# marbl/parsnp

Measured on AMD Instinct MI355X. Metric: genomes/sec (MUM+LCB end-to-end), higher is better.
Workload: dtype int32

## Files before the change

### parsnp_amd/csrc/engine/kernels.h

```cpp
#pragma once
#include <cstdint>

#if defined(__HIPCC__)
#define PM_HD __host__ __device__ inline
#else
#define PM_HD inline
#endif

namespace pm {

PM_HD int ctz64(uint64_t x) {
#if defined(__HIP_DEVICE_COMPILE__)
    return __ffsll((unsigned long long)x) - 1;
#else
    return __builtin_ctzll(x);
#endif
}
PM_HD int clz64(uint64_t x) {
#if defined(__HIP_DEVICE_COMPILE__)
    return __clzll((long long)x);
#else
    return __builtin_clzll(x);
#endif
}
// ... 844 lines not shown
        uint64_t* ev_count = ev_counters + slice * kSliceStride;
        const uint64_t ev_cap = slice_cap;
        uint64_t* const key_out = ev_key + slice * slice_cap;
        uint64_t* const val_out = ev_val + slice * slice_cap;
        uint64_t bk = kEmpty, bv = 0;
        auto emit = [&](int strand, int32_t l0, int64_t j0, int32_t len) {
            const uint64_t ek = ((((uint64_t)pair << lbits) | (uint64_t)l0) << 1) | (uint64_t)strand;
            const uint64_t evv = ((uint64_t)j0 << 32) | (uint32_t)len;
            if (bk == kEmpty) { bk = ek; bv = evv; }
            else { const uint64_t at = atomic_add64(ev_count, 1); if (at < ev_cap) { key_out[at] = ek; val_out[at] = evv; } }
        };
        auto reverse_seed = [&](int64_t j, int32_t l) {
            const int64_t jr = m - K - j;
            const int64_t qpr = rec.qbase_r + jr;
            int32_t lim = (int32_t)(jr < l ? jr : l);
            if (lim > stride) lim = stride;
            const int32_t left = lce_bwd(P, qpr, rbase + l, lim);
            if (left >= stride) return;
            const int32_t rep_l0 = rep[ri.posbase + l - left];
            const int32_t rr = ri.nR - l - K;
            const int32_t maxr = (int32_t)(j < rr ? j : rr);
            const int32_t right = lce_fwd(P, qpr + K, rbase + l + K, maxr);
            const int32_t len = left + K + right;
            if (len >= ri.minlen && len > rep_l0) emit(1, l - left, jr - left, len);
        };
        auto forward_seed = [&](int64_t j, int32_t l) {
            int32_t lim = (int32_t)(j < l ? j : l);
            if (lim > stride) lim = stride;
            const int32_t left = lce_bwd(P, qbase + j, rbase + l, lim);
            if (left >= stride) return;
            const int32_t rep_l0 = rep[ri.posbase + l - left];
            const int64_t mr = m - j - K; const int32_t rr = ri.nR - l - K;
            const int32_t maxr = (int32_t)(mr < rr ? mr : rr);
            const int32_t right = lce_fwd64(P, qbase + j + K, rbase + l + K, maxr);
            const int32_t len = left + K + right;
            if (len >= ri.minlen && len > rep_l0) emit(0, l - left, j - left, len);
        };
        auto walk = [&](int64_t j, uint64_t tag, uint64_t gat, uint64_t slot, int32_t skip, uint64_t head_rt) {
            const bool multi = (slot & kMulti) != 0;
            const int32_t head = slot_head(slot);
            for (int32_t l = head; l >= 0; l = multi ? next[ri.posbase + l] : -1) {
                if (++work > budget) { atomic_or32(err, kErrWork); dense[rec.region] = 1; return; }
                if (l == skip) continue;
                const uint64_t rt = l == head ? head_rt : kmer_tag(P, rbase + l, K);
                if (rt == tag) forward_seed(j, l);
                if (rt == gat) reverse_seed(j, l);
            }
        };
        auto probe_sample = [&](int64_t j, uint64_t tag, uint64_t gat) {
            const uint64_t ctag = gat < tag ? gat : tag;
            uint64_t slot = index_probe(ri, slots, filter, ctag);
            if (slot == kEmpty) return;
            uint64_t rt = kmer_tag(P, rbase + slot_head(slot), K);
            if (rt != tag && rt != gat) {
                slot = index_lookup(P, ri, slots, filter, ctag);
                if (slot == kEmpty) return;
                rt = kmer_tag(P, rbase + slot_head(slot), K);
            }
            walk(j, tag, gat, slot, -1, rt);
        };

        if (live) {
            const int64_t j = (int64_t)it.sample * stride;
            if (it.l >= 0) reverse_seed(j, it.l);
            else if (!dense[rec.region]) {
                const uint64_t tg = kmer_tag(P, qbase + j, K);
                probe_sample(j, tg, rc_tag(tg, K));
            }
        }
        const uint64_t at = wave_reserve01(ev_count, bk != kEmpty);
        if (bk != kEmpty && at < ev_cap) { key_out[at] = bk; val_out[at] = bv; }
    }
};

PM_HD uint64_t even_bits(uint64_t x) {
    x &= 0x5555555555555555ull;
    x = (x | (x >> 1)) & 0x3333333333333333ull;
    x = (x | (x >> 2)) & 0x0f0f0f0f0f0f0f0full;
    x = (x | (x >> 4)) & 0x00ff00ff00ff00ffull;
    x = (x | (x >> 8)) & 0x0000ffff0000ffffull;
    x = (x | (x >> 16)) & 0x00000000ffffffffull;
    return x;
}
PM_HD void planes64(const SeqBlock* blk, int64_t p, uint64_t* b0, uint64_t* b1, uint64_t* nm) {
    const SeqBlock* b = blk + (p >> 5);
    const int sh = (int)(p & 31);
    const SeqBlock x0 = b[0], x1 = b[1], x2 = b[2];
    const uint64_t lo = (x0.b2 >> (2 * sh)) | ((x1.b2 << 1) << (63 - 2 * sh));
    const uint64_t hi = (x1.b2 >> (2 * sh)) | ((x2.b2 << 1) << (63 - 2 * sh));
    *b0 = even_bits(lo) | (even_bits(hi) << 32);
    *b1 = even_bits(lo >> 1) | (even_bits(hi >> 1) << 32);
    const uint64_t m01 = (uint64_t)x0.nm | ((uint64_t)x1.nm << 32);
    *nm = (m01 >> sh) | (((uint64_t)x2.nm << 1) << (63 - sh));
}
struct W64 {
    uint64_t v;
    static PM_HD W64 load(const SeqBlock* blk, int64_t p, int plane) {
        uint64_t b0, b1, nm; planes64(blk, p, &b0, &b1, &nm);
        W64 w; w.v = plane == 0 ? b0 : plane == 1 ? b1 : nm; return w;
    }
    static PM_HD W64 ones(int n) { W64 w; w.v = n >= 64 ? ~0ull : ((1ull << n) - 1); return w; }
    PM_HD W64 shr(int k) const { W64 w; w.v = v >> k; return w; }
    PM_HD W64 operator^(const W64& o) const { W64 w; w.v = v ^ o.v; return w; }
    PM_HD W64 operator|(const W64& o) const { W64 w; w.v = v | o.v; return w; }
    PM_HD W64 operator&(const W64& o) const { W64 w; w.v = v & o.v; return w; }
    PM_HD W64 operator~() const { W64 w; w.v = ~v; return w; }
    PM_HD bool any() const { return v != 0; }
    PM_HD int low() const { return ctz64(v); }
    PM_HD int run_at(int s) const { const uint64_t t = ~(v >> s); return t ? ctz64(t) : 64 - s; }
    PM_HD W64 clear_below(int k) const { W64 w; w.v = k >= 64 ? 0 : v & (~0ull << k); return w; }
    static constexpr int kBits = 64;
};
struct W128 {
    uint64_t lo, hi;
    static PM_HD W128 load(const SeqBlock* blk, int64_t p, int plane) {
        uint64_t a0, a1, an, c0, c1, cn; planes64(blk, p, &a0, &a1, &an); planes64(blk, p + 64, &c0, &c1, &cn);
        W128 w; w.lo = plane == 0 ? a0 : plane == 1 ? a1 : an; w.hi = plane == 0 ? c0 : plane == 1 ? c1 : cn; return w;
    }
    static PM_HD W128 ones(int n) {
        W128 w;
        w.lo = n >= 64 ? ~0ull : ((1ull << n) - 1);
        w.hi = n >= 128 ? ~0ull : n > 64 ? ((1ull << (n - 64)) - 1) : 0;
        return w;
    }
    PM_HD W128 shr(int k) const {
        W128 w;
        if (k >= 64) { w.lo = k >= 128 ? 0 : hi >> (k - 64); w.hi = 0; }
        else { w.lo = (lo >> k) | ((hi << 1) << (63 - k)); w.hi = hi >> k; }
        return w;
    }
    PM_HD W128 operator^(const W128& o) const { W128 w; w.lo = lo ^ o.lo; w.hi = hi ^ o.hi; return w; }
    PM_HD W128 operator|(const W128& o) const { W128 w; w.lo = lo | o.lo; w.hi = hi | o.hi; return w; }
    PM_HD W128 operator&(const W128& o) const { W128 w; w.lo = lo & o.lo; w.hi = hi & o.hi; return w; }
    PM_HD W128 operator~() const { W128 w; w.lo = ~lo; w.hi = ~hi; return w; }
    PM_HD bool any() const { return (lo | hi) != 0; }
    PM_HD int low() const { return lo ? ctz64(lo) : 64 + ctz64(hi); }
    PM_HD int run_at(int s) const { const W128 t = ~shr(s); return t.any() ? t.low() : 128 - s; }
    PM_HD W128 clear_below(int k) const {
        W128 w;
        if (k >= 128) { w.lo = 0; w.hi = 0; }
        else if (k >= 64) { w.lo = 0; w.hi = hi & (~0ull << (k - 64)); }
        else { w.lo = lo & (~0ull << k); w.hi = hi; }
        return w;
    }
    static constexpr int kBits = 128;
};

template <class W, class Emit>
PM_HD void pair_diagonals(const Packed& P, int64_t rpos, int64_t qpos, int32_t nR, int32_t m, int32_t L, Emit emit, int32_t first = 0, int32_t step = 1) {
    const W r0 = W::load(P.blk, rpos, 0), r1 = W::load(P.blk, rpos, 1), rn = W::load(P.blk, rpos, 2);
    const W q0 = W::load(P.blk, qpos, 0), q1 = W::load(P.blk, qpos, 1), qn = W::load(P.blk, qpos, 2);
    const W vr = W::ones(nR), vq = W::ones(m);
    for (int32_t d = -(m - L) + first; d <= nR - L; d += step) {
        W eq;
        if (d >= 0) eq = ~((r0.shr(d) ^ q0) | (r1.shr(d) ^ q1) | (rn.shr(d) ^ qn)) & vr.shr(d) & vq;
        else eq = ~((r0 ^ q0.shr(-d)) | (r1 ^ q1.shr(-d)) | (rn ^ qn.shr(-d))) & vr & vq.shr(-d);
        W x = eq;
        int k = 1;
        while (2 * k <= L) { x = x & x.shr(k); k *= 2; }
        if (L > k) x = x & x.shr(L - k);
        if (!x.any()) continue;
        while (eq.any()) {
            const int s = eq.low();
            const int len = eq.run_at(s);
            if (len >= L) emit(d >= 0 ? s + d : s, d >= 0 ? s : s - d, len);
            eq = eq.clear_below(s + len);
        }
    }
}
struct SmallPairEvents {
    Packed P; const RegionInfo* R; const int64_t* starts; const int64_t* lens; int32_t ngen;
    const int32_t* rep;
    uint64_t* ev_key; uint64_t* ev_val; uint64_t* ev_counters; uint64_t slice_cap; int lbits;
    int32_t g_first, g_last;
    const uint8_t* grouped;

    template <class W, class Emit>
    PM_HD void scan(int64_t rpos, int64_t qpos, int32_t nR, int32_t m, int32_t L, Emit emit) const { pair_diagonals<W>(P, rpos, qpos, nR, m, L, emit); }

    PM_HD void operator()(int64_t tid) const {
        const int64_t pair = tid >> 1; const int strand = (int)(tid & 1);
        const int32_t nq = ngen - 1;
        const int64_t r = pair / nq; const int g = (int)(pair % nq) + 1;
        const RegionInfo& ri = R[r];
        const bool mine = !(grouped && grouped[r]);
        const int64_t m = mine ? lens[r * ngen + g] : 0, qs = mine ? starts[r * ngen + g] : 0;
        const int32_t nR = ri.nR, L = ri.minlen;
        const uint64_t slice = (uint64_t)((tid >> 8) & (kSlices - 1));
        uint64_t* ev_count = ev_counters + slice * kSliceStride;
        uint64_t* const key_out = ev_key + slice * slice_cap;
        uint64_t* const val_out = ev_val + slice * slice_cap;
        uint64_t first_key = kEmpty, first_val = 0;
        if (mine && small_pair(nR, m) && m >= L && nR >= L && g >= g_first && g < g_last) {
            const int64_t qbase = strand ? P.goff[2 * g + 1] + (P.glen[g] - qs - m) : P.goff[2 * g] + qs;
            const int64_t rbase = P.goff[0] + ri.ref_pos;
            auto emit = [&](int32_t l0, int32_t j0, int32_t len) {
                if (len <= rep[ri.posbase + l0]) return;
                const uint64_t ek = ((((uint64_t)pair << lbits) | (uint64_t)l0) << 1) | (uint64_t)strand;
                const uint64_t evv = ((uint64_t)j0 << 32) | (uint32_t)len;
                if (first_key == kEmpty) { first_key = ek; first_val = evv; }
                else { const uint64_t at = atomic_add64(ev_count, 1); if (at < slice_cap) { key_out[at] = ek; val_out[at] = evv; } }
            };
            if (nR <= 64 && m <= 64) scan<W64>(rbase, qbase, nR, (int32_t)m, L, emit);
            else scan<W128>(rbase, qbase, nR, (int32_t)m, L, emit);
        }
        const uint64_t at = wave_reserve01(ev_count, first_key != kEmpty);
        if (first_key != kEmpty && at < slice_cap) { key_out[at] = first_key; val_out[at] = first_val; }
    }
};

struct SliceOffsets {
    const uint64_t* counters; int64_t* off;
    PM_HD void wave(int64_t) const {
#if defined(__HIP_DEVICE_COMPILE__)
        const int lane = (int)__lane_id();
        constexpr int per = kSlices / 64;
        int64_t c[per]; int64_t sum = 0;
        for (int i = 0; i < per; i++) { c[i] = (int64_t)counters[(size_t)(lane * per + i) * kSliceStride]; sum += c[i]; }
        int64_t run = wave_incl_sum64(sum) - sum;
        for (int i = 0; i < per; i++) { off[lane * per + i] = run; run += c[i]; }
        if (lane == 63) off[kSlices] = run;
#else
        int64_t run = 0;
        for (int i = 0; i < kSlices; i++) { off[i] = run; run += (int64_t)counters[(size_t)i * kSliceStride]; }
        off[kSlices] = run;
#endif
    }
};
struct CompactEvents {
    const uint64_t* key_in; const uint64_t* val_in; const int64_t* off; uint64_t slice_cap; uint64_t* key_out; uint64_t* val_out;
    PM_HD void operator()(int64_t tid) const {
        int64_t sl = upper_slot(off, kSlices, tid);
        int64_t src = sl * (int64_t)slice_cap + (tid - off[sl]);
        key_out[tid] = key_in[src]; val_out[tid] = val_in[src];
    }
};

struct PairBucketBase {
    int32_t nq; const int64_t* cbase; int64_t* pbase;
    PM_HD void operator()(int64_t pair) const {
        const int64_t r = pair / nq; const int64_t g = pair % nq;
        pbase[pair] = (int64_t)nq * (cbase[r] - r) + g * (cbase[r + 1] - cbase[r] - 1);
    }
};
PM_HD int64_t bucket_of_key(uint64_t k, int lbits, const int64_t* pbase) {
    return pbase[k >> (lbits + 1)] + (int64_t)(((k >> 1) & ((1ull << lbits) - 1)) >> 8);
}
struct EventBucketCount {
    const uint64_t* key_in; const uint64_t* counters; uint64_t slice_cap; int shift; int lbits; const int64_t* pbase; int64_t* count;
    PM_HD void operator()(int64_t tid) const {
        const uint64_t sl = (uint64_t)tid >> shift, idx = (uint64_t)tid & ((1ull << shift) - 1);
// ... 695 lines not shown
```

### parsnp_amd/csrc/engine/store_kernels.h

```cpp
#pragma once
#include "kernels.h"

namespace pm {

#if defined(__HIP_DEVICE_COMPILE__)
template <class F> __device__ inline void lanes_for(int from, int n, F f) {
    for (int j = (from & ~63) + (int)__lane_id(); j < n; j += 64) if (j >= from) f(j);
}
__device__ inline int32_t wave_min_i32(int32_t x) { for (int d = 32; d >= 1; d >>= 1) { const int32_t y = __shfl_xor(x, d, 64); if (y < x) x = y; } return x; }
__device__ inline int32_t wave_max_i32(int32_t x) { for (int d = 32; d >= 1; d >>= 1) { const int32_t y = __shfl_xor(x, d, 64); if (y > x) x = y; } return x; }
__device__ inline uint32_t wave_or_u32(uint32_t x) { for (int d = 32; d >= 1; d >>= 1) x |= (uint32_t)__shfl_xor((int)x, d, 64); return x; }
__device__ inline int32_t wave_bcast_i32(int32_t x, int lane) { return __shfl(x, lane, 64); }
__device__ inline uint64_t wave_or_u64(uint64_t x) { return ((uint64_t)wave_or_u32((uint32_t)(x >> 32)) << 32) | wave_or_u32((uint32_t)x); }
__device__ inline uint64_t wave_sum_u64(uint64_t x) {
    for (int d = 32; d >= 1; d >>= 1) x += ((uint64_t)(uint32_t)__shfl_xor((int)(x >> 32), d, 64) << 32) | (uint32_t)__shfl_xor((int)(uint32_t)x, d, 64);
    return x;
}
__device__ inline bool wave_leader() { return __lane_id() == 0; }
__device__ inline void wave_sync() { __syncthreads(); }
#define PM_WAVE_SHARED __shared__
__device__ inline uint64_t load_coherent64(const uint64_t* p) { return __hip_atomic_load(p, __ATOMIC_RELAXED, __HIP_MEMORY_SCOPE_AGENT); }
__device__ inline int32_t load_coherent32(const int32_t* p) { return __hip_atomic_load(p, __ATOMIC_RELAXED, __HIP_MEMORY_SCOPE_AGENT); }
__device__ inline uint8_t load_coherent8(const uint8_t* p) { return __hip_atomic_load(p, __ATOMIC_RELAXED, __HIP_MEMORY_SCOPE_AGENT); }
__device__ inline void store_coherent32(int32_t* p, int32_t v) { __hip_atomic_store(p, v, __ATOMIC_RELAXED, __HIP_MEMORY_SCOPE_AGENT); }
// ... 540 lines not shown
        const int64_t i = xcd_item(w, rows);
        if (i >= rows || i >= *nacc || !keep[i]) return;
        const int64_t c = acc[i];
        const int32_t dl = S.shift[c], len = S.len[c];
        const int n = S.ngen;
        int64_t slot = off[i];
        for (int side = 0; side < 2; side++) {
            if (!(keep[i] & (1 << side))) continue;
            if ((uint64_t)slot >= cap) return;
            int64_t rs, rl;
            const int32_t smin = region_extent(S, L, P, c, dl, len, side, &rs, &rl);
            lanes_for(0, n, [&](int j) {
                int64_t a, b;
                region_side(S, L, P, c, dl, len, side, j, &a, &b);
                rg_start[slot * n + j] = a; rg_len[slot * n + j] = b - a;
            });
            if (wave_leader()) info[slot] = RegInfo{2 * i + side, rs, rl, smin, (int32_t)c};
            slot++;
        }
    }
};
constexpr int kAlgPairs = 256;
constexpr int kAlgSets = 64;
struct AlgBytes {
    const RegionInfo* R; const int64_t* lens; int32_t ngen; int64_t npairs; uint64_t* out;
    PM_HD void wave(int64_t w) const {
        uint64_t a = 0, k = 0, q = 0;
        lanes_for(0, kAlgPairs, [&](int t) {
            const int64_t pair = w * kAlgPairs + t;
            if (pair >= npairs) return;
            const int64_t r = pair / (ngen - 1); const int g = (int)(pair % (ngen - 1)) + 1;
            const RegionInfo& ri = R[r];
            const int64_t m = lens[r * ngen + g], n = ri.nR;
            a += (uint64_t)(65 * m + 64 * n);
            k += (uint64_t)m + (g == 1 ? (uint64_t)n : 0ull);
            if (!(m <= 128 && n <= 128) && m >= ri.K && n >= ri.K) k += 16ull * (uint64_t)((m - ri.K) / ri.stride + 1);
            q += (uint64_t)m;
        });
        a = wave_sum_u64(a); k = wave_sum_u64(k); q = wave_sum_u64(q);
        uint64_t* set = out + (size_t)(w & (kAlgSets - 1)) * 8;
        if (wave_leader()) { atomic_add64(set, a); atomic_add64(set + 1, k); atomic_add64(set + 2, q); }
    }
};
struct GatherRegions {
    const int32_t* ids; int32_t ngen; const int64_t* rg_start; const int64_t* rg_len; int64_t* starts; int64_t* lens;
    PM_HD void operator()(int64_t tid) const {
        const int64_t r = ids[tid / ngen]; const int j = (int)(tid % ngen);
        starts[tid] = rg_start[r * ngen + j]; lens[tid] = rg_len[r * ngen + j];
    }
};
struct RegionsEqual {
    const int32_t* a; const int32_t* b; int32_t ngen; const int64_t* rg_start; const int64_t* rg_len; uint8_t* same;
    PM_HD void wave(int64_t i) const {
        const int64_t x = a[i], y = b[i];
        uint32_t diff = 0;
        lanes_for(0, ngen, [&](int j) { if (rg_start[x * ngen + j] != rg_start[y * ngen + j] || rg_len[x * ngen + j] != rg_len[y * ngen + j]) diff = 1; });
        diff = wave_or_u32(diff);
        if (wave_leader()) same[i] = diff ? 0 : 1;
    }
};

#ifndef PM_GRP_EVENTS
#define PM_GRP_EVENTS 8
#endif
constexpr int kGrpEvents = PM_GRP_EVENTS;
constexpr int kGrpPieces = 32;
constexpr int kGrpGenomes = 1024;
struct GroupedPairEvents {
    Packed P; const RegionInfo* R; const int64_t* starts; const int64_t* lens; int32_t ngen; const int32_t* rep;
    uint64_t* ev_key; uint64_t* ev_val; uint64_t* block_count; uint64_t ev_cap; int lbits; int64_t* glo; int32_t g_first, g_last;
    uint8_t* flag;
    EventAtK* st; int32_t* emax;
    int32_t* epm;
    int64_t nreg;
    PM_HD void wave(int64_t w) const {
        const int64_t r = xcd_item(w, nreg);
        if (r >= nreg) return;
        const int32_t nq = ngen - 1;
        const int per = (nq + 63) / 64;
        const RegionInfo& ri = R[r];
        const int32_t nR = ri.nR, L = ri.minlen;
        const int64_t rbase = P.goff[0] + ri.ref_pos;
        uint32_t big = nR > 128 ? 1u : 0u;
        lanes_for(1, ngen, [&](int g) { if (lens[r * ngen + g] > 128) big = 1; });
        big = wave_or_u32(big);
        if (big) { if (wave_leader()) flag[r] = 0; return; }
        PM_WAVE_SHARED uint64_t sh_pl[64][6];
        PM_WAVE_SHARED int32_t sh_m[64];
        PM_WAVE_SHARED uint8_t sh_open[64];
        PM_WAVE_SHARED uint64_t rp_pl[kGrpPieces][6];
        PM_WAVE_SHARED int32_t rp_m[kGrpPieces];
        PM_WAVE_SHARED int32_t rp_g[kGrpPieces];
        PM_WAVE_SHARED uint8_t sh_piece[kGrpGenomes];
        PM_WAVE_SHARED uint32_t sh_ev[2 * kGrpPieces][kGrpEvents];
        PM_WAVE_SHARED int32_t sh_cnt[2 * kGrpPieces];
        PM_WAVE_SHARED uint32_t sh_st[2 * kGrpPieces][kGrpEvents];
        PM_WAVE_SHARED uint8_t sh_used[kGrpPieces];
        PM_WAVE_SHARED int32_t sh_tot[64];
        PM_WAVE_SHARED int32_t sh_elect;
        PM_WAVE_SHARED int32_t sh_bad;
        PM_WAVE_SHARED uint64_t sh_base;
        if (wave_leader()) sh_bad = 0;
        lanes_for(0, kGrpPieces, [&](int i) { sh_used[i] = 0; });
        int npieces = 0;
        for (int k = 0; k < per; k++) {
            wave_sync();
            lanes_for(0, 64, [&](int t) {
                const int g = 1 + t * per + k;
                int32_t m = -1;
                if (g < ngen) {
                    m = (int32_t)lens[r * ngen + g];
                    const int64_t qpos = P.goff[2 * g] + starts[r * ngen + g];
                    const W128 v = W128::ones(m);
                    for (int pl = 0; pl < 3; pl++) { const W128 x = W128::load(P.blk, qpos, pl) & v; sh_pl[t][2 * pl] = x.lo; sh_pl[t][2 * pl + 1] = x.hi; }
                }
                sh_m[t] = m;
                uint8_t open = m >= 0;
                for (int i = 0; i < npieces && open; i++) {
                    if (rp_m[i] != m) continue;
                    bool same = true;
                    for (int x = 0; x < 6 && same; x++) same = rp_pl[i][x] == sh_pl[t][x];
                    if (same) { sh_piece[g - 1] = (uint8_t)i; open = 0; }
                }
                sh_open[t] = open;
            });
            for (;;) {
                wave_sync();
                if (wave_leader()) sh_elect = 64;
                wave_sync();
                lanes_for(0, 64, [&](int t) { if (sh_open[t]) lds_min32(&sh_elect, t); });
                wave_sync();
                const int e = sh_elect;
                if (e == 64) break;
                if (npieces == kGrpPieces) { if (wave_leader()) sh_bad = 1; break; }
                lanes_for(0, 64, [&](int t) {
                    if (t != e) return;
                    for (int x = 0; x < 6; x++) rp_pl[npieces][x] = sh_pl[t][x];
                    rp_m[npieces] = sh_m[t]; rp_g[npieces] = 1 + t * per + k;
                });
                wave_sync();
                lanes_for(0, 64, [&](int t) {
                    if (!sh_open[t] || rp_m[npieces] != sh_m[t]) return;
                    bool same = true;
                    for (int x = 0; x < 6 && same; x++) same = rp_pl[npieces][x] == sh_pl[t][x];
                    if (same) { sh_piece[t * per + k] = (uint8_t)npieces; sh_open[t] = 0; }
                });
                npieces++;
            }
            wave_sync();
            if (sh_bad) break;
        }
        const int tasks = 2 * npieces;
        int share = 1;
        while (share * 2 * tasks <= 64) share *= 2;
        if (!sh_bad) {
            lanes_for(0, tasks, [&](int wi) { sh_cnt[wi] = 0; });
            wave_sync();
            lanes_for(0, tasks * share, [&](int t) {
                const int wi = t / share, sub = t % share;
                const int g = rp_g[wi >> 1], strand = wi & 1;
                const int32_t m = rp_m[wi >> 1];
                if (m < L || nR < L) return;
                const int64_t qs = starts[r * ngen + g];
                const int64_t qbase = strand ? P.goff[2 * g + 1] + (P.glen[g] - qs - m) : P.goff[2 * g] + qs;
                auto emit = [&](int32_t l0, int32_t j0, int32_t len) {
                    if (len <= rep[ri.posbase + l0]) return;
                    const int32_t at = lds_add32(&sh_cnt[wi], 1);
                    if (at < kGrpEvents) sh_ev[wi][at] = (uint32_t)l0 | ((uint32_t)j0 << 8) | ((uint32_t)len << 16);
                };
                if (nR <= 64 && m <= 64) pair_diagonals<W64>(P, rbase, qbase, nR, m, L, emit, sub, share);
                else pair_diagonals<W128>(P, rbase, qbase, nR, m, L, emit, sub, share);
            });
            wave_sync();
            lanes_for(0, tasks, [&](int wi) {
                const int n = sh_cnt[wi];
                if (n > kGrpEvents) { sh_bad = 1; return; }
                for (int i = 1; i < n; i++) {
                    const uint32_t e = sh_ev[wi][i];
                    int at = i;
                    while (at > 0 && (sh_ev[wi][at - 1] & 0xffu) > (e & 0xffu)) { sh_ev[wi][at] = sh_ev[wi][at - 1]; at--; }
                    sh_ev[wi][at] = e;
                }
            });
        }
        wave_sync();
        if (sh_bad) { if (wave_leader()) flag[r] = 0; return; }
        lanes_for(0, tasks, [&](int wi) {
            const int n = sh_cnt[wi];
            int32_t e1 = 0, e2 = 0, wl = 0, wj = 0, up = 0; bool have = false;
            for (int i = 0; i < n; i++) {
                const uint32_t e = sh_ev[wi][i];
                const int32_t l = (int32_t)(e & 0xffu), j = (int32_t)((e >> 8) & 0xffu), end = l + (int32_t)(e >> 16);
                const bool take = !have || end > e1 || (end == e1 && (l < wl || (l == wl && j < wj)));
                if (take) { if (have && e1 > e2) e2 = e1; e1 = end; wl = l; wj = j; up = l + rep[ri.posbase + l]; have = true; }
                else if (end > e2) e2 = end;
                sh_st[wi][i] = (uint32_t)e1 | ((uint32_t)(e2 > up ? e2 : up) << 8) | ((uint32_t)(wj - wl + 128) << 16);
            }
        });
        lanes_for(0, 64, [&](int t) {
            int c = 0;
            for (int k = 0; k < per; k++) {
                const int g = 1 + t * per + k;
                if (g < ngen && g >= g_first && g < g_last) { const int i = sh_piece[g - 1]; c += sh_cnt[2 * i] + sh_cnt[2 * i + 1]; sh_used[i] = 1; }
            }
            sh_tot[t] = c;
        });
        wave_sync();
        lanes_for(0, nR, [&](int k) {
            int32_t ep = nR;
            for (int i = 0; i < npieces; i++) {
                if (!sh_used[i]) continue;
                int32_t v = 0;
                for (int sd = 0; sd < 2; sd++) {
                    const int wi = 2 * i + sd, n = sh_cnt[wi];
                    int32_t e = 0;
                    for (int x = 0; x < n && (int32_t)(sh_ev[wi][x] & 0xffu) <= k; x++) e = (int32_t)(sh_st[wi][x] & 0xffu);
                    if (e > v) v = e;
                }
                if (v < ep) ep = v;
            }
            epm[ri.posbase + k] = ep;
        });
        if (wave_leader()) {
            int total = 0;
            for (int t = 0; t < 64; t++) { const int c = sh_tot[t]; sh_tot[t] = total; total += c; }
            sh_base = total ? atomic_add64(block_count, (uint64_t)total) : 0;
            flag[r] = 1;
        }
        wave_sync();
        lanes_for(0, 64, [&](int t) {
            uint64_t at0 = sh_base + (uint64_t)sh_tot[t];
            for (int k = 0; k < per; k++) {
                const int g = 1 + t * per + k;
                if (g >= ngen) break;
                const int64_t pair = r * nq + (g - 1);
                glo[pair] = (int64_t)at0;
                if (g < g_first || g >= g_last) continue;
                const int i = sh_piece[g - 1];
                const uint32_t* a = sh_ev[2 * i]; const uint32_t* b = sh_ev[2 * i + 1];
                const int na = sh_cnt[2 * i], nb = sh_cnt[2 * i + 1], c = na + nb;
                if (at0 + (uint64_t)c <= ev_cap) {
                    int ia = 0, ib = 0;
                    for (int x = 0; x < c; x++) {
                        const bool fwd = ib >= nb || (ia < na && (a[ia] & 0xffu) <= (b[ib] & 0xffu));
                        const uint32_t e = fwd ? a[ia++] : b[ib++];
                        ev_key[at0 + x] = ((((uint64_t)pair << lbits) | (uint64_t)(e & 0xffu)) << 1) | (fwd ? 0ull : 1ull);
                        ev_val[at0 + x] = ((uint64_t)((e >> 8) & 0xffu) << 32) | (uint64_t)(e >> 16);
                        const uint32_t sf = ia ? sh_st[2 * i][ia - 1] : 0, sr = ib ? sh_st[2 * i + 1][ib - 1] : 0;
                        EventAtK o;
                        o.s[0] = sf ? StrandAtK{(int32_t)(sf & 0xffu), (int32_t)((sf >> 8) & 0xffu), (int32_t)(sf >> 16) - 128} : StrandAtK{0, 0, 0};
                        o.s[1] = sr ? StrandAtK{(int32_t)(sr & 0xffu), (int32_t)((sr >> 8) & 0xffu), (int32_t)(sr >> 16) - 128} : StrandAtK{0, 0, 0};
                        st[at0 + x] = o;
                        emax[at0 + x] = o.s[0].e1 > o.s[1].e1 ? o.s[0].e1 : o.s[1].e1;
                    }
                }
                at0 += (uint64_t)c;
            }
        });
    }
};
struct GroupedBounds {
    const uint8_t* flag; const int64_t* glo; int32_t nq; int64_t* lo;
    PM_HD void operator()(int64_t pair) const { if (flag[pair / nq]) lo[pair] = glo[pair]; }
};

constexpr int kWideEvents = 32;
constexpr int kWidePieces = 128;
constexpr int kWideGenomes = 2047;
struct GroupedPairEventsWide {
    Packed P; const RegionInfo* R; const int64_t* starts; const int64_t* lens; int32_t ngen; const int32_t* rep;
    uint64_t* ev_key; uint64_t* ev_val; uint64_t* block_count; uint64_t ev_cap; int lbits; int64_t* glo; int32_t g_first, g_last;
    uint8_t* flag;
    EventAtK* st; int32_t* emax; int32_t* epm;
    int64_t nreg;
    int after_first;
    uint64_t* wide;
    PM_HD void wave(int64_t w) const {
        const int64_t r = xcd_item(w, nreg);
        if (r >= nreg) return;
        if (after_first && flag[r]) return;
        const int32_t nq = ngen - 1;
        const int per = (nq + 63) / 64;
        const RegionInfo& ri = R[r];
        const int32_t nR = ri.nR, L = ri.minlen;
        const int64_t rbase = P.goff[0] + ri.ref_pos;
        uint32_t big = nR > 128 || nq > kWideGenomes ? 1u : 0u;
        lanes_for(1, ngen, [&](int g) { if (lens[r * ngen + g] > 128) big = 1; });
        big = wave_or_u32(big);
        if (big) { if (wave_leader()) flag[r] = 0; return; }
        PM_WAVE_SHARED uint64_t sh_pl[64][6];
        PM_WAVE_SHARED int32_t sh_m[64];
        PM_WAVE_SHARED uint8_t sh_open[64];
        PM_WAVE_SHARED uint64_t rp_pl[kWidePieces][6];
        PM_WAVE_SHARED int32_t rp_m[kWidePieces];
        PM_WAVE_SHARED int32_t rp_g[kWidePieces];
        PM_WAVE_SHARED uint8_t sh_piece[kWideGenomes + 1];
        PM_WAVE_SHARED uint32_t sh_ev[2 * kWidePieces][kWideEvents];
        PM_WAVE_SHARED int32_t sh_cnt[2 * kWidePieces];
        PM_WAVE_SHARED uint8_t sh_used[kWidePieces];
        PM_WAVE_SHARED int32_t sh_tot[64];
        PM_WAVE_SHARED int32_t sh_elect;
        PM_WAVE_SHARED int32_t sh_bad;
        PM_WAVE_SHARED uint64_t sh_base;
        if (wave_leader()) sh_bad = 0;
        lanes_for(0, kWidePieces, [&](int i) { sh_used[i] = 0; });
        int npieces = 0;
        bool bad = false;
        for (int k = 0; k < per && !bad; k++) {
            wave_sync();
            lanes_for(0, 64, [&](int t) {
                const int g = 1 + t * per + k;
                int32_t m = -1;
                if (g < ngen) {
                    m = (int32_t)lens[r * ngen + g];
                    const int64_t qpos = P.goff[2 * g] + starts[r * ngen + g];
                    const W128 v = W128::ones(m);
                    for (int pl = 0; pl < 3; pl++) { const W128 x = W128::load(P.blk, qpos, pl) & v; sh_pl[t][2 * pl] = x.lo; sh_pl[t][2 * pl + 1] = x.hi; }
                }
                sh_m[t] = m;
                uint8_t open = m >= 0;
                for (int i = 0; i < kWidePieces; i++) {
                    if (i >= npieces || !open) break;
                    if (rp_m[i] != m) continue;
                    bool same = true;
                    for (int x = 0; x < 6; x++) same = same && rp_pl[i][x] == sh_pl[t][x];
                    if (same) { sh_piece[g - 1] = (uint8_t)i; open = 0; }
                }
                sh_open[t] = open;
            });
            for (int round = 0; round < 65; round++) {
                wave_sync();
                if (wave_leader()) sh_elect = 64;
                wave_sync();
                lanes_for(0, 64, [&](int t) { if (sh_open[t]) lds_min32(&sh_elect, t); });
                wave_sync();
                const int e = sh_elect;
                if (e == 64) break;
                if (npieces == kWidePieces) { if (wave_leader()) sh_bad = 1; break; }
                lanes_for(0, 64, [&](int t) {
                    if (t != e) return;
// ... 1077 lines not shown
```

Before: 31370.

## Restructure grouped pair-events kernel: register planes, prefetch, LDS reuse, parallel output write

The grouped small-region event kernel now keeps each lane's query bit-planes in registers instead of LDS, and software-prefetches the next genome's sequence blocks. Diagonal scanning reuses the cached distinct-piece planes, deriving the reverse strand by bit reversal instead of reloading from global memory. The reference planes are loaded once, and repeat thresholds are staged into an LDS byte table. The event output loop now precomputes the merge order per piece and writes one event per lane using a wave prefix sum and binary search, replacing the serial per-lane merge. This adds complexity and relies on repeat values clamped to 255 and on correct bit-reversal equivalence for reverse strands.

```diff
diff --git a/parsnp_amd/csrc/engine/kernels.h b/parsnp_amd/csrc/engine/kernels.h
--- a/parsnp_amd/csrc/engine/kernels.h
+++ b/parsnp_amd/csrc/engine/kernels.h
@@ -950,16 +950,17 @@
     x = (x | (x >> 16)) & 0x00000000ffffffffull;
     return x;
 }
-PM_HD void planes64(const SeqBlock* blk, int64_t p, uint64_t* b0, uint64_t* b1, uint64_t* nm) {
-    const SeqBlock* b = blk + (p >> 5);
-    const int sh = (int)(p & 31);
-    const SeqBlock x0 = b[0], x1 = b[1], x2 = b[2];
+PM_HD void planes64_of(const SeqBlock& x0, const SeqBlock& x1, const SeqBlock& x2, int sh, uint64_t* b0, uint64_t* b1, uint64_t* nm) {
     const uint64_t lo = (x0.b2 >> (2 * sh)) | ((x1.b2 << 1) << (63 - 2 * sh));
     const uint64_t hi = (x1.b2 >> (2 * sh)) | ((x2.b2 << 1) << (63 - 2 * sh));
     *b0 = even_bits(lo) | (even_bits(hi) << 32);
     *b1 = even_bits(lo >> 1) | (even_bits(hi >> 1) << 32);
     const uint64_t m01 = (uint64_t)x0.nm | ((uint64_t)x1.nm << 32);
     *nm = (m01 >> sh) | (((uint64_t)x2.nm << 1) << (63 - sh));
+}
+PM_HD void planes64(const SeqBlock* blk, int64_t p, uint64_t* b0, uint64_t* b1, uint64_t* nm) {
+    const SeqBlock* b = blk + (p >> 5);
+    planes64_of(b[0], b[1], b[2], (int)(p & 31), b0, b1, nm);
 }
 struct W64 {
     uint64_t v;
@@ -1015,10 +1016,8 @@
 };
 
 template <class W, class Emit>
-PM_HD void pair_diagonals(const Packed& P, int64_t rpos, int64_t qpos, int32_t nR, int32_t m, int32_t L, Emit emit, int32_t first = 0, int32_t step = 1) {
-    const W r0 = W::load(P.blk, rpos, 0), r1 = W::load(P.blk, rpos, 1), rn = W::load(P.blk, rpos, 2);
-    const W q0 = W::load(P.blk, qpos, 0), q1 = W::load(P.blk, qpos, 1), qn = W::load(P.blk, qpos, 2);
-    const W vr = W::ones(nR), vq = W::ones(m);
+PM_HD void pair_diagonals(const W& r0, const W& r1, const W& rn, const W& q0, const W& q1, const W& qn, const W& vr, const W& vq,
+                          int32_t nR, int32_t m, int32_t L, Emit emit, int32_t first = 0, int32_t step = 1) {
     for (int32_t d = -(m - L) + first; d <= nR - L; d += step) {
         W eq;
         if (d >= 0) eq = ~((r0.shr(d) ^ q0) | (r1.shr(d) ^ q1) | (rn.shr(d) ^ qn)) & vr.shr(d) & vq;
@@ -1035,6 +1034,32 @@
             eq = eq.clear_below(s + len);
         }
     }
+}
+template <class W, class Emit>
+PM_HD void pair_diagonals(const Packed& P, int64_t rpos, int64_t qpos, int32_t nR, int32_t m, int32_t L, Emit emit, int32_t first = 0, int32_t step = 1) {
+    const W r0 = W::load(P.blk, rpos, 0), r1 = W::load(P.blk, rpos, 1), rn = W::load(P.blk, rpos, 2);
+    const W q0 = W::load(P.blk, qpos, 0), q1 = W::load(P.blk, qpos, 1), qn = W::load(P.blk, qpos, 2);
+    pair_diagonals<W>(r0, r1, rn, q0, q1, qn, W::ones(nR), W::ones(m), nR, m, L, emit, first, step);
+}
+PM_HD uint64_t rev_bits64(uint64_t x) {
+#if defined(__HIP_DEVICE_COMPILE__)
+    return (uint64_t)__brevll((unsigned long long)x);
+#else
+    x = ((x >> 1) & 0x5555555555555555ull) | ((x & 0x5555555555555555ull) << 1);
+    x = ((x >> 2) & 0x3333333333333333ull) | ((x & 0x3333333333333333ull) << 2);
+    x = ((x >> 4) & 0x0f0f0f0f0f0f0f0full) | ((x & 0x0f0f0f0f0f0f0f0full) << 4);
+    return __builtin_bswap64(x);
+#endif
+}
+PM_HD W128 reversed_bits(const W128& x, int32_t m) {
+    W128 w; w.lo = rev_bits64(x.hi); w.hi = rev_bits64(x.lo);
+    return w.shr(128 - m);
+}
+PM_HD void reverse_strand_planes(W128* b0, W128* b1, W128* nm, int32_t m) {
+    const W128 n = reversed_bits(*nm, m), keep = ~n & W128::ones(m);
+    *b0 = ~reversed_bits(*b0, m) & keep;
+    *b1 = ~reversed_bits(*b1, m) & keep;
+    *nm = n;
 }
 struct SmallPairEvents {
     Packed P; const RegionInfo* R; const int64_t* starts; const int64_t* lens; int32_t ngen;
diff --git a/parsnp_amd/csrc/engine/store_kernels.h b/parsnp_amd/csrc/engine/store_kernels.h
--- a/parsnp_amd/csrc/engine/store_kernels.h
+++ b/parsnp_amd/csrc/engine/store_kernels.h
@@ -646,68 +646,111 @@
         const int32_t nR = ri.nR, L = ri.minlen;
         const int64_t rbase = P.goff[0] + ri.ref_pos;
         uint32_t big = nR > 128 ? 1u : 0u;
-        lanes_for(1, ngen, [&](int g) { if (lens[r * ngen + g] > 128) big = 1; });
+        lanes_for(1, ngen, [&](int g) { const int64_t m = lens[r * ngen + g]; if (m > 128) big |= 1; if (m > 64) big |= 2; });
         big = wave_or_u32(big);
-        if (big) { if (wave_leader()) flag[r] = 0; return; }
-        PM_WAVE_SHARED uint64_t sh_pl[64][6];
-        PM_WAVE_SHARED int32_t sh_m[64];
-        PM_WAVE_SHARED uint8_t sh_open[64];
-        PM_WAVE_SHARED uint64_t rp_pl[kGrpPieces][6];
+        if (big & 1) { if (wave_leader()) flag[r] = 0; return; }
+        const bool upper = (big & 2) != 0;
+#if defined(__HIP_DEVICE_COMPILE__)
+        constexpr int kOwn = 1;
+        auto own = [](int) { return 0; };
+#else
+        constexpr int kOwn = 64;
+        auto own = [](int t) { return t; };
+#endif
+        uint64_t own_pl[kOwn][6];
+        int32_t own_m[kOwn];
+        uint8_t own_open[kOwn];
+        PM_WAVE_SHARED union Tables {
+            uint64_t pl[kGrpPieces][6];
+            struct Block {
+                uint8_t mg[kGrpPieces][2 * kGrpEvents];
+                uint16_t off[65];
+            } b;
+        } rp_u;
+        static_assert(sizeof(Tables) == sizeof(uint64_t) * kGrpPieces * 6, "the tables of step 3 must fit the space of the distinct pieces");
+        static_assert(kGrpEvents < 0x80 && kGrpGenomes * 2 * kGrpEvents <= 0xffff, "mg is a byte, off 16 bits");
         PM_WAVE_SHARED int32_t rp_m[kGrpPieces];
-        PM_WAVE_SHARED int32_t rp_g[kGrpPieces];
         PM_WAVE_SHARED uint8_t sh_piece[kGrpGenomes];
         PM_WAVE_SHARED uint32_t sh_ev[2 * kGrpPieces][kGrpEvents];
         PM_WAVE_SHARED int32_t sh_cnt[2 * kGrpPieces];
         PM_WAVE_SHARED uint32_t sh_st[2 * kGrpPieces][kGrpEvents];
         PM_WAVE_SHARED uint8_t sh_used[kGrpPieces];
-        PM_WAVE_SHARED int32_t sh_tot[64];
         PM_WAVE_SHARED int32_t sh_elect;
         PM_WAVE_SHARED int32_t sh_bad;
         PM_WAVE_SHARED uint64_t sh_base;
+        PM_WAVE_SHARED uint8_t sh_rep[128];
         if (wave_leader()) sh_bad = 0;
         lanes_for(0, kGrpPieces, [&](int i) { sh_used[i] = 0; });
+        lanes_for(0, nR, [&](int k) { const int32_t v = rep[ri.posbase + k]; sh_rep[k] = (uint8_t)(v > 255 ? 255 : v < 0 ? 0 : v); });
         int npieces = 0;
+        struct Fetch { int32_t m; int sh; SeqBlock b[5]; };
+        auto fetch = [&](int t, int k) {
+            Fetch f = {}; f.m = -1;
+            const int g = 1 + t * per + k;
+            if (g < ngen) {
+                f.m = (int32_t)lens[r * ngen + g];
+                const int64_t qpos = P.goff[2 * g] + starts[r * ngen + g];
+                const SeqBlock* b = P.blk + (qpos >> 5);
+                f.sh = (int)(qpos & 31);
+                f.b[0] = b[0]; f.b[1] = b[1]; f.b[2] = b[2];
+                if (upper) { f.b[3] = b[3]; f.b[4] = b[4]; }
+            }
+            return f;
+        };
+#if defined(__HIP_DEVICE_COMPILE__)
+        Fetch ahead = fetch((int)__lane_id(), 0);
+#endif
         for (int k = 0; k < per; k++) {
             wave_sync();
+#if defined(__HIP_DEVICE_COMPILE__)
+            const Fetch now = ahead;
+            if (k + 1 < per) ahead = fetch((int)__lane_id(), k + 1);
+#endif
             lanes_for(0, 64, [&](int t) {
+#if defined(__HIP_DEVICE_COMPILE__)
+                const Fetch& f = now;
+#else
+                const Fetch f = fetch(t, k);
+#endif
                 const int g = 1 + t * per + k;
-                int32_t m = -1;
+                const int32_t m = f.m;
                 if (g < ngen) {
-                    m = (int32_t)lens[r * ngen + g];
-                    const int64_t qpos = P.goff[2 * g] + starts[r * ngen + g];
                     const W128 v = W128::ones(m);
-                    for (int pl = 0; pl < 3; pl++) { const W128 x = W128::load(P.blk, qpos, pl) & v; sh_pl[t][2 * pl] = x.lo; sh_pl[t][2 * pl + 1] = x.hi; }
-                }
-                sh_m[t] = m;
+                    uint64_t lo[3], hi[3] = {0, 0, 0};
+                    planes64_of(f.b[0], f.b[1], f.b[2], f.sh, &lo[0], &lo[1], &lo[2]);
+                    if (upper) planes64_of(f.b[2], f.b[3], f.b[4], f.sh, &hi[0], &hi[1], &hi[2]);
+                    for (int pl = 0; pl < 3; pl++) { own_pl[own(t)][2 * pl] = lo[pl] & v.lo; own_pl[own(t)][2 * pl + 1] = hi[pl] & v.hi; }
+                }
+                own_m[own(t)] = m;
                 uint8_t open = m >= 0;
                 for (int i = 0; i < npieces && open; i++) {
                     if (rp_m[i] != m) continue;
                     bool same = true;
-                    for (int x = 0; x < 6 && same; x++) same = rp_pl[i][x] == sh_pl[t][x];
+                    for (int x = 0; x < 6 && same; x++) same = rp_u.pl[i][x] == own_pl[own(t)][x];
                     if (same) { sh_piece[g - 1] = (uint8_t)i; open = 0; }
                 }
-                sh_open[t] = open;
+                own_open[own(t)] = open;
             });
             for (;;) {
                 wave_sync();
                 if (wave_leader()) sh_elect = 64;
                 wave_sync();
-                lanes_for(0, 64, [&](int t) { if (sh_open[t]) lds_min32(&sh_elect, t); });
+                lanes_for(0, 64, [&](int t) { if (own_open[own(t)]) lds_min32(&sh_elect, t); });
                 wave_sync();
                 const int e = sh_elect;
                 if (e == 64) break;
                 if (npieces == kGrpPieces) { if (wave_leader()) sh_bad = 1; break; }
                 lanes_for(0, 64, [&](int t) {
                     if (t != e) return;
-                    for (int x = 0; x < 6; x++) rp_pl[npieces][x] = sh_pl[t][x];
-                    rp_m[npieces] = sh_m[t]; rp_g[npieces] = 1 + t * per + k;
+                    for (int x = 0; x < 6; x++) rp_u.pl[npieces][x] = own_pl[own(t)][x];
+                    rp_m[npieces] = own_m[own(t)];
                 });
                 wave_sync();
                 lanes_for(0, 64, [&](int t) {
-                    if (!sh_open[t] || rp_m[npieces] != sh_m[t]) return;
+                    if (!own_open[own(t)] || rp_m[npieces] != own_m[own(t)]) return;
                     bool same = true;
-                    for (int x = 0; x < 6 && same; x++) same = rp_pl[npieces][x] == sh_pl[t][x];
-                    if (same) { sh_piece[t * per + k] = (uint8_t)npieces; sh_open[t] = 0; }
+                    for (int x = 0; x < 6 && same; x++) same = rp_u.pl[npieces][x] == own_pl[own(t)][x];
+                    if (same) { sh_piece[t * per + k] = (uint8_t)npieces; own_open[own(t)] = 0; }
                 });
                 npieces++;
             }
@@ -720,20 +763,28 @@
         if (!sh_bad) {
             lanes_for(0, tasks, [&](int wi) { sh_cnt[wi] = 0; });
             wave_sync();
+            W128 r0, r1, rn;
+            r0.hi = r1.hi = rn.hi = 0;
+            planes64(P.blk, rbase, &r0.lo, &r1.lo, &rn.lo);
+            if (nR > 64) planes64(P.blk, rbase + 64, &r0.hi, &r1.hi, &rn.hi);
             lanes_for(0, tasks * share, [&](int t) {
                 const int wi = t / share, sub = t % share;
-                const int g = rp_g[wi >> 1], strand = wi & 1;
-                const int32_t m = rp_m[wi >> 1];
+                const int i = wi >> 1, strand = wi & 1;
+                const int32_t m = rp_m[i];
                 if (m < L || nR < L) return;
-                const int64_t qs = starts[r * ngen + g];
-                const int64_t qbase = strand ? P.goff[2 * g + 1] + (P.glen[g] - qs - m) : P.goff[2 * g] + qs;
+                W128 q0, q1, qn;
+                q0.lo = rp_u.pl[i][0]; q0.hi = rp_u.pl[i][1]; q1.lo = rp_u.pl[i][2]; q1.hi = rp_u.pl[i][3]; qn.lo = rp_u.pl[i][4]; qn.hi = rp_u.pl[i][5];
+                if (strand) reverse_strand_planes(&q0, &q1, &qn, m);
                 auto emit = [&](int32_t l0, int32_t j0, int32_t len) {
-                    if (len <= rep[ri.posbase + l0]) return;
+                    if (len <= (int32_t)sh_rep[l0]) return;
                     const int32_t at = lds_add32(&sh_cnt[wi], 1);
                     if (at < kGrpEvents) sh_ev[wi][at] = (uint32_t)l0 | ((uint32_t)j0 << 8) | ((uint32_t)len << 16);
                 };
-                if (nR <= 64 && m <= 64) pair_diagonals<W64>(P, rbase, qbase, nR, m, L, emit, sub, share);
-                else pair_diagonals<W128>(P, rbase, qbase, nR, m, L, emit, sub, share);
+                if (nR <= 64 && m <= 64) {
+                    W64 a0, a1, an, b0, b1, bn;
+                    a0.v = r0.lo; a1.v = r1.lo; an.v = rn.lo; b0.v = q0.lo; b1.v = q1.lo; bn.v = qn.lo;
+                    pair_diagonals<W64>(a0, a1, an, b0, b1, bn, W64::ones(nR), W64::ones(m), nR, m, L, emit, sub, share);
+                } else pair_diagonals<W128>(r0, r1, rn, q0, q1, qn, W128::ones(nR), W128::ones(m), nR, m, L, emit, sub, share);
             });
             wave_sync();
             lanes_for(0, tasks, [&](int wi) {
@@ -756,20 +807,52 @@
                 const uint32_t e = sh_ev[wi][i];
                 const int32_t l = (int32_t)(e & 0xffu), j = (int32_t)((e >> 8) & 0xffu), end = l + (int32_t)(e >> 16);
                 const bool take = !have || end > e1 || (end == e1 && (l < wl || (l == wl && j < wj)));
-                if (take) { if (have && e1 > e2) e2 = e1; e1 = end; wl = l; wj = j; up = l + rep[ri.posbase + l]; have = true; }
+                if (take) { if (have && e1 > e2) e2 = e1; e1 = end; wl = l; wj = j; up = l + (int32_t)sh_rep[l]; have = true; }
                 else if (end > e2) e2 = end;
                 sh_st[wi][i] = (uint32_t)e1 | ((uint32_t)(e2 > up ? e2 : up) << 8) | ((uint32_t)(wj - wl + 128) << 16);
             }
         });
-        lanes_for(0, 64, [&](int t) {
+        lanes_for(0, npieces, [&](int i) {
+            const uint32_t* a = sh_ev[2 * i]; const uint32_t* b = sh_ev[2 * i + 1];
+            const int na = sh_cnt[2 * i], nb = sh_cnt[2 * i + 1];
+            int ia = 0, ib = 0;
+            for (int x = 0; x < 2 * kGrpEvents; x++) {
+                if (x >= na + nb) break;
+                const bool fwd = ib >= nb || (ia < na && (a[ia] & 0xffu) <= (b[ib] & 0xffu));
+                if (fwd) ia++; else ib++;
+                rp_u.b.mg[i][x] = (uint8_t)(ia | (fwd ? 0x80 : 0));
+            }
+        });
+        auto count_of = [&](int g) { const int i = sh_piece[g - 1]; return sh_cnt[2 * i] + sh_cnt[2 * i + 1]; };
+#if defined(__HIP_DEVICE_COMPILE__)
+        {
+            const int t = (int)__lane_id();
             int c = 0;
             for (int k = 0; k < per; k++) {
                 const int g = 1 + t * per + k;
-                if (g < ngen && g >= g_first && g < g_last) { const int i = sh_piece[g - 1]; c += sh_cnt[2 * i] + sh_cnt[2 * i + 1]; sh_used[i] = 1; }
-            }
-            sh_tot[t] = c;
-        });
+                if (g < ngen && g >= g_first && g < g_last) { c += count_of(g); sh_used[sh_piece[g - 1]] = 1; }
+            }
+            const int incl = wave_incl_sum(c);
+            rp_u.b.off[t] = (uint16_t)(incl - c);
+            if (t == 63) rp_u.b.off[64] = (uint16_t)incl;
+        }
+#else
+        {
+            int at = 0;
+            for (int t = 0; t < 64; t++) {
+                rp_u.b.off[t] = (uint16_t)at;
+                for (int k = 0; k < per; k++) {
+                    const int g = 1 + t * per + k;
+                    if (g < ngen && g >= g_first && g < g_last) { at += count_of(g); sh_used[sh_piece[g - 1]] = 1; }
+                }
+            }
+            rp_u.b.off[64] = (uint16_t)at;
+        }
+#endif
         wave_sync();
+        const int total = rp_u.b.off[64];
+        uint64_t reserved = 0;
+        if (wave_leader() && total) reserved = atomic_add64(block_count, (uint64_t)total);
         lanes_for(0, nR, [&](int k) {
             int32_t ep = nR;
             for (int i = 0; i < npieces; i++) {
@@ -785,41 +868,49 @@
             }
             epm[ri.posbase + k] = ep;
         });
-        if (wave_leader()) {
-            int total = 0;
-            for (int t = 0; t < 64; t++) { const int c = sh_tot[t]; sh_tot[t] = total; total += c; }
-            sh_base = total ? atomic_add64(block_count, (uint64_t)total) : 0;
-            flag[r] = 1;
-        }
+        if (wave_leader()) { sh_base = reserved; flag[r] = 1; }
         wave_sync();
+        const uint64_t base = sh_base;
         lanes_for(0, 64, [&](int t) {
-            uint64_t at0 = sh_base + (uint64_t)sh_tot[t];
+            int at = rp_u.b.off[t];
             for (int k = 0; k < per; k++) {
                 const int g = 1 + t * per + k;
                 if (g >= ngen) break;
-                const int64_t pair = r * nq + (g - 1);
-                glo[pair] = (int64_t)at0;
-                if (g < g_first || g >= g_last) continue;
-                const int i = sh_piece[g - 1];
-                const uint32_t* a = sh_ev[2 * i]; const uint32_t* b = sh_ev[2 * i + 1];
-                const int na = sh_cnt[2 * i], nb = sh_cnt[2 * i + 1], c = na + nb;
-                if (at0 + (uint64_t)c <= ev_cap) {
-                    int ia = 0, ib = 0;
-                    for (int x = 0; x < c; x++) {
-                        const bool fwd = ib >= nb || (ia < na && (a[ia] & 0xffu) <= (b[ib] & 0xffu));
-                        const uint32_t e = fwd ? a[ia++] : b[ib++];
-                        ev_key[at0 + x] = ((((uint64_t)pair << lbits) | (uint64_t)(e & 0xffu)) << 1) | (fwd ? 0ull : 1ull);
-                        ev_val[at0 + x] = ((uint64_t)((e >> 8) & 0xffu) << 32) | (uint64_t)(e >> 16);
-                        const uint32_t sf = ia ? sh_st[2 * i][ia - 1] : 0, sr = ib ? sh_st[2 * i + 1][ib - 1] : 0;
-                        EventAtK o;
-                        o.s[0] = sf ? StrandAtK{(int32_t)(sf & 0xffu), (int32_t)((sf >> 8) & 0xffu), (int32_t)(sf >> 16) - 128} : StrandAtK{0, 0, 0};
-                        o.s[1] = sr ? StrandAtK{(int32_t)(sr & 0xffu), (int32_t)((sr >> 8) & 0xffu), (int32_t)(sr >> 16) - 128} : StrandAtK{0, 0, 0};
-                        st[at0 + x] = o;
-                        emax[at0 + x] = o.s[0].e1 > o.s[1].e1 ? o.s[0].e1 : o.s[1].e1;
-                    }
-                }
-                at0 += (uint64_t)c;
-            }
+                glo[r * nq + (g - 1)] = (int64_t)(base + (uint64_t)at);
+                if (g >= g_first && g < g_last) at += count_of(g);
+            }
+        });
+        lanes_for(0, total, [&](int x0) {
+            int t = 0, hi = 64;
+            for (int s = 0; s < 6; s++) {
+                const int mid = (t + hi) >> 1;
+                if ((int)rp_u.b.off[mid] <= x0) t = mid; else hi = mid;
+            }
+            int at = rp_u.b.off[t], q = -1, c = 0;
+            for (int k = 0; k < per; k++) {
+                const int g = 1 + t * per + k;
+                if (g >= ngen) break;
+                c = g >= g_first && g < g_last ? count_of(g) : 0;
+                if (x0 < at + c) { q = g - 1; break; }
+                at += c;
+            }
+            if (q < 0) return;
+            if (base + (uint64_t)(at + c) > ev_cap) return;
+            const int64_t pair = r * nq + q;
+            const int i = sh_piece[q], x = x0 - at;
+            const uint32_t w = rp_u.b.mg[i][x];
+            const bool fwd = (w & 0x80u) != 0;
+            const int ia = (int)(w & 0x7fu), ib = x + 1 - ia;
+            const uint32_t e = fwd ? sh_ev[2 * i][ia - 1] : sh_ev[2 * i + 1][ib - 1];
+            const uint64_t dst = base + (uint64_t)x0;
+            ev_key[dst] = ((((uint64_t)pair << lbits) | (uint64_t)(e & 0xffu)) << 1) | (fwd ? 0ull : 1ull);
+            ev_val[dst] = ((uint64_t)((e >> 8) & 0xffu) << 32) | (uint64_t)(e >> 16);
+            const uint32_t sf = ia ? sh_st[2 * i][ia - 1] : 0, sr = ib ? sh_st[2 * i + 1][ib - 1] : 0;
+            EventAtK o;
+            o.s[0] = sf ? StrandAtK{(int32_t)(sf & 0xffu), (int32_t)((sf >> 8) & 0xffu), (int32_t)(sf >> 16) - 128} : StrandAtK{0, 0, 0};
+            o.s[1] = sr ? StrandAtK{(int32_t)(sr & 0xffu), (int32_t)((sr >> 8) & 0xffu), (int32_t)(sr >> 16) - 128} : StrandAtK{0, 0, 0};
+            st[dst] = o;
+            emax[dst] = o.s[0].e1 > o.s[1].e1 ? o.s[0].e1 : o.s[1].e1;
         });
     }
 };
```

After: 30800. 0.982x the previous value.
